# purejade/pinot

Measured on AMD Instinct MI355X. Metric: rows/sec for filter+group-by SUM at 1/2/4/8 GPUs; % of HBM roofline, higher is better.
Workload: dtype int64; 1 GPU; c5: BASELINE configs[4]: 4096 x 2M rows sharded over the GPUs, (f1 IN 32 ids OR f2=7) AND f3<>3, group by gk (card 1000), sum(m); segments=4096, rows_total=8192000000, parallelism=dp1 (segment sharding)

## Files before the change

### pinot_amd/csrc/pgx_roaring.hip

```cpp
#include <hip/hip_runtime.h>
#include <stdint.h>

#include <algorithm>

#include "pgx_device.h"
#include "pgx_internal.h"
#include "pgx_roaring_device.h"

namespace pgx {

__device__ __forceinline__ const PGX_G JRDesc* gdescs(const RDesc* descs) { return (const PGX_G JRDesc*)descs; }

__device__ __forceinline__ PgxRLeavesReg<1> one_leaf(const RDesc* descs, int a) {
  PgxRLeavesReg<1> L;
  L.desc[0] = a;
  L.b0[0] = 0;
  L.total = a >= 0 ? descs[a].nb : 0;
  return L;
}

__global__ void __launch_bounds__(256) pgx_roaring_expand(const RDesc* __restrict__ descs, int npairs, int maxchunks) {
  const int pair = static_cast<int>(blockIdx.x / maxchunks);
  const int chunk = static_cast<int>(blockIdx.x - static_cast<unsigned>(pair) * maxchunks);
  if (pair >= npairs) return;
  const RDesc& D = descs[pair];
  if (chunk >= D.nchunks) return;
  __shared__ uint32_t m[2048];
  __shared__ PgxRScratch S;
  const int tid = threadIdx.x;
  pgx_rexpand<256>(one_leaf(descs, pair), gdescs(descs), chunk, m, S);
  uint32_t* out = D.mask + static_cast<size_t>(chunk) * 2048;
  for (int i = tid; i < 2048; i += 256) out[i] = m[i];
}

constexpr int kRProgStack = 4;
__global__ void __launch_bounds__(256) pgx_roaring_program(const RProg* __restrict__ progs, const RDesc* __restrict__ descs,
                                                           int nprogs, int maxchunks) {
  const int pi = static_cast<int>(blockIdx.x / maxchunks);
  const int chunk = static_cast<int>(blockIdx.x - static_cast<unsigned>(pi) * maxchunks);
  if (pi >= nprogs) return;
  const RProg& P = progs[pi];
  if (chunk >= P.nchunks) return;
  __shared__ uint32_t stk[kRProgStack][2048];
  __shared__ PgxRScratch S;
  const int tid = threadIdx.x;
  const int64_t doc0 = static_cast<int64_t>(chunk) << 16;
  int sp = 0;
  for (int i = 0; i < P.nops; ++i) {
    const int op = P.op[i];
    if (op == RP_LEAF) {
      pgx_rexpand<256>(one_leaf(descs, P.arg[i]), gdescs(descs), chunk, stk[sp], S);
      ++sp;
    } else if (op == RP_NOT) {
      uint32_t* m = stk[sp - 1];
      for (int w = tid; w < 2048; w += 256) m[w] = ~m[w] & pgx_rkeep(doc0 + 32 * w, P.num_docs);
    } else {
      uint32_t* a = stk[sp - 2];
      const uint32_t* b = stk[sp - 1];
      for (int w = tid; w < 2048; w += 256) a[w] = op == RP_AND ? (a[w] & b[w]) : (a[w] | b[w]);
      --sp;
    }
    __syncthreads();
  }
  uint32_t* out = P.mask + static_cast<size_t>(chunk) * 2048;
  for (int w = tid; w < 2048; w += 256) out[w] = stk[0][w];
}

constexpr int kRProgMaxLeaves = PGX_J_MAX_RLEAVES;
__device__ __forceinline__ uint32_t rprog_word(const RProg& P, const uint32_t* lm, int chunk, int w) {
  uint32_t st[kRProgMaxLeaves];
  int sp = 0, leaf = 0;
  const uint32_t keep = pgx_rkeep((static_cast<int64_t>(chunk) << 16) + 32 * w, P.num_docs);
  for (int i = 0; i < P.nops; ++i) {
    const int op = P.op[i];
    if (op == RP_LEAF) {
      st[sp++] = lm[leaf * 2048 + w];
      ++leaf;
    } else if (op == RP_NOT) {
      st[sp - 1] = ~st[sp - 1] & keep;
    } else {
      st[sp - 2] = op == RP_AND ? (st[sp - 2] & st[sp - 1]) : (st[sp - 2] | st[sp - 1]);
      --sp;
    }
  }
  return st[0];
}

__global__ void __launch_bounds__(256) pgx_roaring_program_wide(const RProg* __restrict__ progs,
                                                                const RDesc* __restrict__ descs, int nprogs,
                                                                int maxchunks) {
  const int pi = static_cast<int>(blockIdx.x / maxchunks);
  const int chunk = static_cast<int>(blockIdx.x - static_cast<unsigned>(pi) * maxchunks);
  if (pi >= nprogs) return;
  const RProg& P = progs[pi];
  if (chunk >= P.nchunks) return;
  extern __shared__ uint32_t lmask[];
  __shared__ PgxRScratch S;
  __shared__ int leaf_desc[kRProgMaxLeaves], leaf_b0[kRProgMaxLeaves + 1], nleaves;
  const int tid = threadIdx.x;
  if (tid == 0) {
    int nl = 0, tot = 0;
    for (int i = 0; i < P.nops; ++i)
      if (P.op[i] == RP_LEAF) {
        const int a = P.arg[i];
        leaf_desc[nl] = a;
        leaf_b0[nl] = tot;
        tot += a >= 0 ? descs[a].nb : 0;
        ++nl;
      }
    leaf_b0[nl] = tot;
    nleaves = nl;
  }
  __syncthreads();
  const PgxRLeavesLds L{leaf_desc, leaf_b0, nleaves, leaf_b0[nleaves]};
  pgx_rexpand<256>(L, gdescs(descs), chunk, lmask, S);
  __syncthreads();
  uint32_t* out = P.mask + static_cast<size_t>(chunk) * 2048;
  for (int w = tid; w < 2048; w += 256) out[w] = rprog_word(P, lmask, chunk, w);
}

constexpr int kSegRThreads = 512;
constexpr int kSegRBitmaps = 512;
__global__ void __launch_bounds__(kSegRThreads, 8) pgx_roaring_program_seg(const RProg* __restrict__ progs,
                                                                        const RDesc* __restrict__ descs, int nprogs,
                                                                        int parts) {
  const int pi = static_cast<int>(blockIdx.x) / parts;
  if (pi >= nprogs) return;
  const RProg& P = progs[pi];
  const int per = (P.nchunks + parts - 1) / parts;
  const int c0 = (static_cast<int>(blockIdx.x) % parts) * per;
  const int c1 = min(P.nchunks, c0 + per);
  if (c0 >= c1) return;
  extern __shared__ uint32_t lmask[];
  __shared__ const uint8_t* cptr[kSegRBitmaps];
  __shared__ int ccard[kSegRBitmaps], cpre[kSegRBitmaps + 1], cleaf[kSegRBitmaps];
  __shared__ int ncont;
  __shared__ int bidx[kSegRBitmaps], nbm;
  const int tid = threadIdx.x;
  int nl = 0, tot = 0, leaf = 0, my_desc = -1, my_first = 0;
  for (int i = 0; i < P.nops; ++i)
    if (P.op[i] == RP_LEAF && nl < kRProgMaxLeaves) {
      const int a = P.arg[i];
      const int nb = a >= 0 ? descs[a].nb : 0;
      if (tid >= tot && tid < tot + nb) {
        leaf = nl;
        my_desc = a;
        my_first = tot;
      }
      tot += nb;
      ++nl;
    }
  PgxRCursor cu;
  if (my_desc >= 0) cu.seek(pgx_rbitmap(gdescs(descs) + my_desc, tid - my_first), c0);
  constexpr int kPer = 4;
  for (int chunk = c0; chunk < c1; ++chunk) {
    for (int i = tid; i < nl * 2048; i += kSegRThreads) lmask[i] = 0u;
    if (tid == 0) ncont = 0;
    pgx_lds_barrier();
    if (cu.key == chunk) {
      const int slot = atomicAdd(&ncont, 1);
      cptr[slot] = cu.ptr();
      ccard[slot] = cu.card;
      cleaf[slot] = leaf;
      cu.advance();
    }
    pgx_lds_barrier();
    const int nc = ncont;
    if (tid < 64) pgx_rcard_prefix<kSegRBitmaps / 64, true>(tid, nc, ccard, cpre, &cpre[kSegRBitmaps], bidx, &nbm);
    pgx_lds_barrier();
    const int ne = cpre[kSegRBitmaps];
    const int nbc = nbm;
    uint32_t bw[2048 / kSegRThreads];
    if (nbc > 0) pgx_rwords_load<kSegRThreads>(cptr[bidx[0]], tid, bw);
    pgx_rspread<kSegRThreads, kPer>(tid, nc, ne, cptr, cpre, cleaf, lmask);
    for (int i = 0; i < nbc; ++i) {
      const int k = bidx[i];
      if (i > 0) pgx_rwords_load<kSegRThreads>(cptr[k], tid, bw);
      pgx_rwords_or<kSegRThreads>(lmask + cleaf[k] * 2048, tid, bw);
    }
    pgx_lds_barrier();
    uint32_t* out = P.mask + static_cast<size_t>(chunk) * 2048;
    for (int w = tid; w < 2048; w += kSegRThreads) out[w] = rprog_word(P, lmask, chunk, w);
    pgx_lds_barrier();
  }
}

#ifndef PGX_WAVE_ELEMS
#define PGX_WAVE_ELEMS 16
#endif

template <int NS, int WPB, int MINW>
__global__ void __launch_bounds__(64 * WPB, MINW) pgx_roaring_program_wave(const RProg* __restrict__ progs,
                                                                          const RDesc* __restrict__ descs, int nprogs,
                                                                          int parts) {
  extern __shared__ uint32_t wmask[];
  __shared__ int wpre[WPB][65];
  __shared__ const uint8_t* wptr[WPB][64];
  __shared__ int wslot[WPB][64];
  const int lane = static_cast<int>(threadIdx.x) & 63, wv = static_cast<int>(threadIdx.x) >> 6;
  const int gw = static_cast<int>(blockIdx.x) * WPB + wv;
  const int pi = gw / parts;
  if (pi >= nprogs) return;
  const RProg& P = progs[pi];
  const int per = (P.nchunks + parts - 1) / parts;
  const int c0 = (gw % parts) * per;
  const int c1 = min(P.nchunks, c0 + per);
  if (c0 >= c1) return;
  uint32_t* sm = wmask + wv * NS * 2048;
  int* pre = wpre[wv];
  const uint8_t** ptrs = wptr[wv];
  int* slots = wslot[wv];
  int my_desc = -1, my_first = 0, my_slot = 0, my_phase = 0;
  bool any_andnot = false;
  {
    RPlan plan;
    int tot = 0;
    for (int i = 0; i < P.nops;) {
      const bool is_leaf = P.op[i] == RP_LEAF;
      const int a = P.arg[i];
      i += plan.step(P, i);
      if (!is_leaf) continue;
      const int nb = a >= 0 ? descs[a].nb : 0;
      if (lane >= tot && lane < tot + nb) {
        my_desc = a;
        my_first = tot;
        my_slot = plan.slot;
        my_phase = plan.phase;
      }
      tot += nb;
      any_andnot |= plan.phase != 0;
    }
  }
  PgxRCursor cu;
  if (my_desc >= 0) cu.seek(pgx_rbitmap(gdescs(descs) + my_desc, lane - my_first), c0);
#pragma unroll
  for (int s = 0; s < NS; ++s)
    for (int j = 0; j < 32; ++j) sm[s * 2048 + j * 64 + lane] = 0u;
  for (int chunk = c0; chunk < c1; ++chunk) {
    const bool act = cu.key == chunk;
    const uint8_t* cptr = cu.ptr();
    const int ccard = cu.card;
    if (act) cu.advance();
    for (int ph = 0; ph < (any_andnot ? 2 : 1); ++ph) {
      const bool mine = act && my_phase == ph;
      const bool arr = mine && ccard <= 4096;
      const int v = arr ? ccard : 0;
      int incl = v;
#pragma unroll
      for (int d = 1; d < 64; d <<= 1) {
        const int y = __shfl_up(incl, d, 64);
        if (lane >= d) incl += y;
      }
      const int total = __shfl(incl, 63, 64);
      pre[lane] = incl - v;
      if (lane == 63) pre[64] = incl;
      ptrs[lane] = mine ? cptr : nullptr;
      slots[lane] = my_slot;
      uint64_t bm = __ballot(mine && ccard > 4096);
      pgx_wave_lds_sync();
      if (total > 0) {
        int k = 0;
#pragma unroll
        for (int step = 32; step > 0; step >>= 1)
          if (pre[k + step] <= lane) k += step;
        int kend = pre[k + 1], kbeg = pre[k];
        const uint8_t* kp = ptrs[k];
        int ks = slots[k];
        constexpr int B = PGX_WAVE_ELEMS;
        for (int e0 = lane; e0 < total; e0 += 64 * B) {
          uint32_t val[B];
          int dst[B];
#pragma unroll
          for (int q = 0; q < B; ++q) {
            const int e = e0 + 64 * q;
            dst[q] = -1;
            if (e < total) {
              while (kend <= e) {
                ++k;
                kbeg = kend;
                kend = pre[k + 1];
                kp = ptrs[k];
                ks = slots[k];
              }
              val[q] = pgx_rd16(kp + 2 * (e - kbeg));
              dst[q] = ks * 2048;
            }
          }
#pragma unroll
          for (int q = 0; q < B; ++q)
            if (dst[q] >= 0) {
              if (ph == 0) atomicOr(&sm[dst[q] + (val[q] >> 5)], 1u << (val[q] & 31u));
              else atomicAnd(&sm[dst[q] + (val[q] >> 5)], ~(1u << (val[q] & 31u)));
            }
        }
      }
      while (bm) {
        const int src = __builtin_ctzll(bm);
        bm &= bm - 1;
        const uint8_t* c = ptrs[src];
        uint32_t* m = sm + slots[src] * 2048;
        const bool al = (reinterpret_cast<uintptr_t>(c) & 3u) == 0;
#pragma unroll 1
        for (int h = 0; h < 2; ++h) {
          uint32_t x[16];
          if (al) {
            const PGX_G uint32_t* c32 = (const PGX_G uint32_t*)(c);
#pragma unroll
            for (int j = 0; j < 16; ++j) x[j] = c32[(h * 16 + j) * 64 + lane];
          } else {
#pragma unroll
            for (int j = 0; j < 16; ++j) x[j] = pgx_rd32(c + 4 * ((h * 16 + j) * 64 + lane));
          }
#pragma unroll
          for (int j = 0; j < 16; ++j)
            if (x[j]) {
              if (ph == 0) atomicOr(&m[(h * 16 + j) * 64 + lane], x[j]);
              else atomicAnd(&m[(h * 16 + j) * 64 + lane], ~x[j]);
            }
        }
      }
      pgx_wave_lds_sync();
    }
    const int64_t doc0 = static_cast<int64_t>(chunk) << 16;
    uint32_t* out = P.mask + static_cast<size_t>(chunk) * 2048;
    RPlan plan;
    for (int i = 0; i < P.nops;) {
      const int op = P.op[i];
      i += plan.step(P, i);
      if (op == RP_LEAF) continue;
      uint32_t* a = sm + plan.slot * 2048;
      if (op == RP_NOT) {
#pragma unroll 4
        for (int j = 0; j < 32; ++j) {
          const int w = j * 64 + lane;
          a[w] = ~a[w] & pgx_rkeep(doc0 + 32 * w, P.num_docs);
        }
      } else {
        const uint32_t* b = sm + plan.rhs * 2048;
        if (op == RP_AND) {
#pragma unroll 8
          for (int j = 0; j < 32; ++j) a[j * 64 + lane] &= b[j * 64 + lane];
        } else {
#pragma unroll 8
          for (int j = 0; j < 32; ++j) a[j * 64 + lane] |= b[j * 64 + lane];
        }
      }
    }
    const uint32_t* r = sm + plan.top() * 2048;
#pragma unroll 8
    for (int j = 0; j < 32; ++j) out[j * 64 + lane] = r[j * 64 + lane];
    for (int s = 0; s < NS; ++s)
#pragma unroll 8
      for (int j = 0; j < 32; ++j) sm[s * 2048 + j * 64 + lane] = 0u;
    pgx_wave_lds_sync();
  }
}

}

extern "C" hipError_t pgx_launch_roaring(const pgx::RDesc* descs, int npairs, int maxchunks, hipStream_t stream) {
  if (npairs <= 0 || maxchunks <= 0) return hipSuccess;
  const long long blocks = static_cast<long long>(npairs) * maxchunks;
  if (blocks > 0x7FFFFFFFll) return hipErrorInvalidValue;
  hipLaunchKernelGGL(pgx::pgx_roaring_expand, dim3(static_cast<unsigned>(blocks)), dim3(256), 0, stream, descs, npairs,
                     maxchunks);
  return hipGetLastError();
}

extern "C" hipError_t pgx_launch_roaring_program_wave(const pgx::RProg* progs, const pgx::RDesc* descs, int nprogs,
                                                      int maxchunks, int nslots, hipStream_t stream) {
  if (nprogs <= 0 || maxchunks <= 0) return hipSuccess;
  int parts = std::max(1, std::min(maxchunks, (8192 + nprogs - 1) / nprogs));
  const long long waves = static_cast<long long>(nprogs) * parts;
#define PGX_WAVE_LAUNCH(NS, WPB, MINW)                                                                             \
  hipLaunchKernelGGL((pgx::pgx_roaring_program_wave<NS, WPB, MINW>),                                              \
                     dim3(static_cast<unsigned>((waves + WPB - 1) / WPB)), dim3(64 * WPB),                        \
                     static_cast<size_t>(NS) * WPB * 2048 * 4, stream, progs, descs, nprogs, parts)
  if (nslots <= 1) PGX_WAVE_LAUNCH(1, 4, 4);
  else if (nslots == 2) PGX_WAVE_LAUNCH(2, 2, 2);
  else PGX_WAVE_LAUNCH(3, 2, 1);
#undef PGX_WAVE_LAUNCH
  return hipGetLastError();
}

extern "C" hipError_t pgx_launch_roaring_program(const pgx::RProg* progs, const pgx::RDesc* descs, int nprogs,
                                                 int maxchunks, int maxleaves, hipStream_t stream) {
  if (nprogs <= 0 || maxchunks <= 0) return hipSuccess;
  const long long blocks = static_cast<long long>(nprogs) * maxchunks;
  if (maxleaves < 0 && -maxleaves <= pgx::kRProgMaxLeaves) {
    int parts = std::max(1, std::min(std::min(maxchunks, 8), (2048 + nprogs - 1) / nprogs));
      hipLaunchKernelGGL(pgx::pgx_roaring_program_seg, dim3(static_cast<unsigned>(nprogs * parts)),
                       dim3(pgx::kSegRThreads), static_cast<size_t>(-maxleaves) * 2048 * 4, stream, progs, descs,
                       nprogs, parts);
    return hipGetLastError();
  }
  if (maxleaves >= 1 && maxleaves <= pgx::kRProgMaxLeaves) {
    hipLaunchKernelGGL(pgx::pgx_roaring_program_wide, dim3(static_cast<unsigned>(blocks)), dim3(256),
                       static_cast<size_t>(maxleaves) * 2048 * 4, stream, progs, descs, nprogs, maxchunks);
    return hipGetLastError();
  }
  hipLaunchKernelGGL(pgx::pgx_roaring_program, dim3(static_cast<unsigned>(blocks)), dim3(256), 0, stream, progs, descs,
                     nprogs, maxchunks);
  return hipGetLastError();
}
```

### pinot_amd/csrc/pgx_roaring_device.h

```cpp
#ifndef PGX_ROARING_DEVICE_H_
#define PGX_ROARING_DEVICE_H_

__device__ __forceinline__ u32 pgx_rd16(const unsigned char* p) { return *(const PGX_G unsigned short*)p; }
__device__ __forceinline__ u32 pgx_rd32(const unsigned char* p) { return pgx_rd16(p) | (pgx_rd16(p + 2) << 16); }
__device__ __forceinline__ const unsigned char* pgx_rbitmap(const PGX_G JRDesc* d, int k) {
  const u32 id = ((const PGX_G u32*)d->ids)[k];
  return d->inv + __builtin_bswap32(((const PGX_G u32*)d->inv)[id]);
}

__device__ __forceinline__ int pgx_rcontainer(const unsigned char* base, int chunk, const unsigned char*& ptr) {
  const int n = (int)pgx_rd32(base + 4);
  int lo = 0, hi = n - 1, found = -1;
  const int g = min(chunk, n - 1);
  if (g >= 0) {
    const int k = (int)pgx_rd16(base + 8 + 4 * g);
    if (k == chunk) found = g;
    else if (k < chunk) lo = g + 1;
    else hi = g - 1;
  }
  while (found < 0 && lo <= hi) {
    const int mid = (lo + hi) >> 1;
    const int k = (int)pgx_rd16(base + 8 + 4 * mid);
    if (k == chunk) { found = mid; break; }
    if (k < chunk) lo = mid + 1; else hi = mid - 1;
  }
  if (found < 0) return 0;
  ptr = base + pgx_rd32(base + 8 + 4 * n + 4 * found);
  return (int)pgx_rd16(base + 8 + 4 * found + 2) + 1;
}

struct PgxRCursor {
  const unsigned char* base = nullptr;
  int n = 0, cur = 0, key = 1 << 30, card = 0;
  u32 off = 0;
  __device__ __forceinline__ void load() {
    int k = 1 << 30, c = card;
    u32 o = off;
    if (cur < n) {
      k = (int)pgx_rd16(base + 8 + 4 * cur);
      c = (int)pgx_rd16(base + 8 + 4 * cur + 2) + 1;
      o = pgx_rd32(base + 8 + 4 * n + 4 * cur);
    }
    key = k, card = c, off = o;
  }
  __device__ __forceinline__ void seek(const unsigned char* bitmap, int c0) {
    base = bitmap;
    n = (int)pgx_rd32(base + 4);
    if (c0 > 0 && n > 0) {
      if (n > c0 && (int)pgx_rd16(base + 8 + 4 * c0) == c0) {
        cur = c0;
      } else {
        int lo = 0, hi = n;
        while (lo < hi) {
          const int mid = (lo + hi) >> 1;
          if ((int)pgx_rd16(base + 8 + 4 * mid) < c0) lo = mid + 1; else hi = mid;
        }
        cur = lo;
      }
    }
    load();
  }
  __device__ __forceinline__ void advance() {
    ++cur;
    load();
  }
  __device__ __forceinline__ const unsigned char* ptr() const { return base + off; }
};

template <int PER, bool LIST>
__device__ __forceinline__ void pgx_rcard_prefix(int lane, int nc, const int* ccard, int* cpre, int* total, int* bidx,
                                                 int* nbm) {
  int v[PER], x = 0, nb = 0;
#pragma unroll
  for (int q = 0; q < PER; ++q) {
    const int k = lane * PER + q;
    const bool in = k < nc;
    v[q] = (in && ccard[k] <= 4096) ? ccard[k] : 0;
    if (LIST) nb += (in && ccard[k] > 4096) ? 1 : 0;
    x += v[q];
  }
  int incl = x, binc = nb;
#pragma unroll
  for (int d = 1; d < 64; d <<= 1) {
    const int y = __shfl_up(incl, d, 64);
    const int z = LIST ? __shfl_up(binc, d, 64) : 0;
    if (lane >= d) {
      incl += y;
      binc += z;
    }
  }
  int e = incl - x, b = binc - nb;
#pragma unroll
  for (int q = 0; q < PER; ++q) {
    const int k = lane * PER + q;
    cpre[k] = e;
    e += v[q];
    if (LIST && k < nc && ccard[k] > 4096) bidx[b++] = k;
  }
  if (lane == 63) {
    *total = incl;
    if (LIST) *nbm = binc;
  }
}

template <int NT, int PER>
__device__ __forceinline__ void pgx_rspread(int tid, int nc, int ne, const unsigned char* const* cptr, const int* cpre,
                                            const int* cleaf, u32* lm) {
  for (int e0 = 0; e0 < ne; e0 += PER * NT) {
    u32 val[PER];
    int dst[PER];
#pragma unroll
    for (int q = 0; q < PER; ++q) {
      const int i = e0 + q * NT + tid, e = min(i, ne - 1);
      int lo = 0, hi = nc - 1;
      while (lo < hi) {
        const int mid = (lo + hi + 1) >> 1;
        if (cpre[mid] <= e) lo = mid; else hi = mid - 1;
      }
      val[q] = pgx_rd16(cptr[lo] + 2 * (e - cpre[lo]));
      dst[q] = i < ne ? cleaf[lo] * 2048 : -1;
    }
#pragma unroll
    for (int q = 0; q < PER; ++q) {
      const bool in = dst[q] >= 0;
      atomicOr(&lm[in ? dst[q] + (val[q] >> 5) : tid], in ? 1u << (val[q] & 31u) : 0u);
    }
  }
}

template <int NT>
__device__ __forceinline__ void pgx_rwords_load(const unsigned char* c, int tid, u32* x) {
#pragma unroll
  for (int q = 0; q < 2048 / NT; ++q) x[q] = pgx_rd32(c + 4 * (q * NT + tid));
}
template <int NT>
__device__ __forceinline__ void pgx_rwords_or(u32* m, int tid, const u32* x) {
#pragma unroll
  for (int q = 0; q < 2048 / NT; ++q)
    if (x[q]) atomicOr(&m[q * NT + tid], x[q]);
}

__device__ __forceinline__ u32 pgx_rkeep(long long d, int num_docs) {
  return d >= num_docs ? 0u : (d + 32 > num_docs ? (1u << (num_docs - d)) - 1u : 0xFFFFFFFFu);
}

#define PGX_RB 256
struct PgxRScratch {
  const unsigned char* cptr[PGX_RB];
  int ccard[PGX_RB], cpre[PGX_RB], cleaf[PGX_RB];
  int ncont, celems;
};

template <int NL>
struct PgxRLeavesReg {
  int desc[NL], b0[NL], total;
  __device__ __forceinline__ int leaves() const { return NL; }
  __device__ __forceinline__ void locate(int b, int& leaf, int& d, int& first) const {
    leaf = 0, d = desc[0], first = 0;
#pragma unroll
    for (int q = 1; q < NL; ++q)
      if (b >= b0[q]) { leaf = q; d = desc[q]; first = b0[q]; }
  }
};
struct PgxRLeavesLds {
  const int* desc;
  const int* b0;
  int nl, total;
  __device__ __forceinline__ int leaves() const { return nl; }
  __device__ __forceinline__ void locate(int b, int& leaf, int& d, int& first) const {
    leaf = 0;
    while (b0[leaf + 1] <= b) ++leaf;
    d = desc[leaf], first = b0[leaf];
  }
};

template <int NT, class LT>
__device__ void pgx_rexpand(const LT& L, const PGX_G JRDesc* D, int chunk, u32* lm, PgxRScratch& S) {
  const int tid = threadIdx.x;
  for (int i = tid; i < L.leaves() * 2048; i += NT) lm[i] = 0u;
  for (int b0 = 0; b0 < L.total; b0 += PGX_RB) {
    if (tid == 0) S.ncont = 0;
    pgx_lds_barrier();
    const int b = b0 + tid;
    if (tid < PGX_RB && b < L.total) {
      int leaf, d, first;
      L.locate(b, leaf, d, first);
      const unsigned char* ptr;
      const int card = pgx_rcontainer(pgx_rbitmap(D + d, b - first), chunk, ptr);
      if (card) {
        const int slot = atomicAdd(&S.ncont, 1);
        S.cptr[slot] = ptr;
        S.ccard[slot] = card;
        S.cleaf[slot] = leaf;
      }
    }
    pgx_lds_barrier();
    const int nc = S.ncont;
    if (tid < 64) pgx_rcard_prefix<PGX_RB / 64, false>(tid, nc, S.ccard, S.cpre, &S.celems, nullptr, nullptr);
    pgx_lds_barrier();
    pgx_rspread<NT, 4>(tid, nc, S.celems, S.cptr, S.cpre, S.cleaf, lm);
    for (int k = 0; k < nc; ++k) {
      if (S.ccard[k] <= 4096) continue;
      u32 x[2048 / NT];
      pgx_rwords_load<NT>(S.cptr[k], tid, x);
      pgx_rwords_or<NT>(lm + S.cleaf[k] * 2048, tid, x);
    }
    pgx_lds_barrier();
  }
}

template <int NT, int NL>
__device__ void pgx_rchunk_leaves(const PGX_G JRProg* P, const PGX_G JRDesc* D, int chunk, u32* lm, PgxRScratch& S) {
  PgxRLeavesReg<NL> L;
  L.total = 0;
#pragma unroll
  for (int j = 0; j < NL; ++j) {
    L.desc[j] = P->ldesc[j];
    L.b0[j] = L.total;
    L.total += L.desc[j] >= 0 ? D[L.desc[j]].nb : 0;
  }
  pgx_rexpand<NT>(L, D, chunk, lm, S);
}

#endif
```

Baseline: 1493 billion rows/s.

## Add wide vectorized path to roaring program wave kernel

Adds a WIDE variant of the per-wave roaring program kernel and makes it the default. Array containers are now read as 16-byte granules with per-lane valid masks, and bitmap containers are loaded as 128-bit vectors and realigned with alignbit and shuffles. The prefix sum uses DPP, and the boolean program is evaluated with vector LDS ops. The cursor packs key and card into a single 32-bit load, and parts is now sized from the device CU count. These changes aim to cut scalar 16-bit loads and per-element overhead in mask construction, at the cost of more complexity and register pressure, plus possible alignment edge cases.

```diff
diff --git a/pinot_amd/csrc/pgx_roaring.hip b/pinot_amd/csrc/pgx_roaring.hip
--- a/pinot_amd/csrc/pgx_roaring.hip
+++ b/pinot_amd/csrc/pgx_roaring.hip
@@ -2,6 +2,8 @@
 #include <stdint.h>
 
 #include <algorithm>
+#include <cstdlib>
+#include <cstring>
 
 #include "pgx_device.h"
 #include "pgx_internal.h"
@@ -157,10 +159,10 @@
     for (int i = tid; i < nl * 2048; i += kSegRThreads) lmask[i] = 0u;
     if (tid == 0) ncont = 0;
     pgx_lds_barrier();
-    if (cu.key == chunk) {
+    if (cu.key() == chunk) {
       const int slot = atomicAdd(&ncont, 1);
       cptr[slot] = cu.ptr();
-      ccard[slot] = cu.card;
+      ccard[slot] = cu.card();
       cleaf[slot] = leaf;
       cu.advance();
     }
@@ -185,20 +187,101 @@
   }
 }
 
-#ifndef PGX_WAVE_ELEMS
-#define PGX_WAVE_ELEMS 16
-#endif
-
-template <int NS, int WPB, int MINW>
+constexpr int kWaveGranules = 7;
+constexpr int kWaveNarrowElems = 16;
+typedef u32 pgx_u32x4_dw __attribute__((ext_vector_type(4), aligned(4)));
+
+template <int B>
+__device__ __forceinline__ void wave_granules_load(int base, int end, int lane, const int* pre,
+                                                   const uint8_t* const* ptrs, const int* meta, pgx_u32x4 (&A)[B],
+                                                   u32 (&am)[B]) {
+#pragma unroll
+  for (int q = 0; q < B; ++q) {
+    const int gi = base + 64 * q + lane, g = min(gi, end - 1);
+    int k = 0;
+#pragma unroll
+    for (int step = 32; step > 0; step >>= 1)
+      if (pre[k + step] <= g) k += step;
+    const uintptr_t s = reinterpret_cast<uintptr_t>(ptrs[k]);
+    const int m = meta[k];
+    const uintptr_t ga = (s & ~static_cast<uintptr_t>(15)) + 16 * static_cast<uintptr_t>(g - pre[k]);
+    A[q] = *(const PGX_G pgx_u32x4*)ga;
+    const int first = max(static_cast<int>(s - ga), 0) >> 1;
+    const int last = min(static_cast<int>(s + 2 * (m & 0xFFFF) - ga), 16) >> 1;
+    const u32 vm = gi < end ? (0xFFu >> (8 - last)) & (0xFFu << first) & 0xFFu : 0u;
+    am[q] = vm | static_cast<u32>(m >> 16) << 8;
+  }
+}
+template <int PH, int B>
+__device__ __forceinline__ void wave_granules_apply(u32* sm, const pgx_u32x4 (&A)[B], const u32 (&am)[B]) {
+#pragma unroll
+  for (int q = 0; q < B; ++q) {
+    u32* d = sm + (am[q] >> 8);
+#pragma unroll
+    for (int i = 0; i < 8; ++i) {
+      const u32 w = A[q][i >> 1];
+      const u32 v = (i & 1) ? w >> 16 : w & 0xFFFFu;
+      if ((am[q] >> i) & 1u) {
+        if (PH == 0) atomicOr(&d[v >> 5], 1u << (v & 31u));
+        else atomicAnd(&d[v >> 5], ~(1u << (v & 31u)));
+      }
+    }
+  }
+}
+template <int J0, int H>
+__device__ __forceinline__ void wave_words_load(uintptr_t c, int lane, pgx_u32x4 (&W)[H], u32& tail) {
+  const PGX_G unsigned char* cb = (const PGX_G unsigned char*)(c & ~static_cast<uintptr_t>(3));
+#pragma unroll
+  for (int j = 0; j < H; ++j) W[j] = *(const PGX_G pgx_u32x4_dw*)(cb + static_cast<u32>(16 * (64 * (J0 + j) + lane)));
+  tail = 0u;
+  if ((c & 2) && lane == 0) tail = *(const PGX_G u32*)(cb + 1024u * (J0 + H));
+}
+template <int PH, int J0, int H>
+__device__ __forceinline__ void wave_words_apply(u32* m, uintptr_t c, int lane, const pgx_u32x4 (&W)[H], u32 tail) {
+  const u32 sh = (c & 2) ? 16u : 0u;
+  pgx_u32x4* m4 = reinterpret_cast<pgx_u32x4*>(m) + 64 * J0 + lane;
+#pragma unroll
+  for (int j = 0; j < H; ++j) {
+    const u32 wrap = __builtin_amdgcn_readfirstlane(j < H - 1 ? W[(j + 1) % H].x : tail);
+    const u32 up = __shfl(W[j].x, (lane + 1) & 63, 64);
+    const u32 next = lane == 63 ? wrap : up;
+    pgx_u32x4 o;
+    o.x = __builtin_amdgcn_alignbit(W[j].y, W[j].x, sh);
+    o.y = __builtin_amdgcn_alignbit(W[j].z, W[j].y, sh);
+    o.z = __builtin_amdgcn_alignbit(W[j].w, W[j].z, sh);
+    o.w = __builtin_amdgcn_alignbit(next, W[j].w, sh);
+    const pgx_u32x4 cur = m4[64 * j];
+    m4[64 * j] = PH == 0 ? (cur | o) : (cur & ~o);
+  }
+}
+__device__ __forceinline__ int wave_prefix_sum(int v) {
+  v += __builtin_amdgcn_update_dpp(0, v, 0x111, 0xF, 0xF, false);
+  v += __builtin_amdgcn_update_dpp(0, v, 0x112, 0xF, 0xF, false);
+  v += __builtin_amdgcn_update_dpp(0, v, 0x114, 0xF, 0xF, false);
+  v += __builtin_amdgcn_update_dpp(0, v, 0x118, 0xF, 0xF, false);
+  v += __builtin_amdgcn_update_dpp(0, v, 0x142, 0xA, 0xF, false);
+  v += __builtin_amdgcn_update_dpp(0, v, 0x143, 0xC, 0xF, false);
+  return v;
+}
+__device__ __forceinline__ int wave_bits_below(uint64_t m) {
+  return static_cast<int>(__builtin_amdgcn_mbcnt_hi(static_cast<u32>(m >> 32), __builtin_amdgcn_mbcnt_lo(static_cast<u32>(m), 0u)));
+}
+__device__ __forceinline__ uintptr_t wave_lane_ptr(uintptr_t v, int src) {
+  const u32 lo = __builtin_amdgcn_readlane(static_cast<u32>(v), src);
+  const u32 hi = __builtin_amdgcn_readlane(static_cast<u32>(v >> 32), src);
+  return (static_cast<uintptr_t>(hi) << 32) | lo;
+}
+
+template <int NS, int WPB, int MINW, bool WIDE>
 __global__ void __launch_bounds__(64 * WPB, MINW) pgx_roaring_program_wave(const RProg* __restrict__ progs,
                                                                           const RDesc* __restrict__ descs, int nprogs,
                                                                           int parts) {
-  extern __shared__ uint32_t wmask[];
+  extern __shared__ __attribute__((aligned(16))) uint32_t wmask[];
   __shared__ int wpre[WPB][65];
   __shared__ const uint8_t* wptr[WPB][64];
   __shared__ int wslot[WPB][64];
   const int lane = static_cast<int>(threadIdx.x) & 63, wv = static_cast<int>(threadIdx.x) >> 6;
-  const int gw = static_cast<int>(blockIdx.x) * WPB + wv;
+  const int gw = __builtin_amdgcn_readfirstlane(static_cast<int>(blockIdx.x) * WPB + wv);
   const int pi = gw / parts;
   if (pi >= nprogs) return;
   const RProg& P = progs[pi];
@@ -207,11 +290,13 @@
   const int c1 = min(P.nchunks, c0 + per);
   if (c0 >= c1) return;
   uint32_t* sm = wmask + wv * NS * 2048;
+  pgx_u32x4* sm4 = reinterpret_cast<pgx_u32x4*>(sm);
   int* pre = wpre[wv];
   const uint8_t** ptrs = wptr[wv];
   int* slots = wslot[wv];
   int my_desc = -1, my_first = 0, my_slot = 0, my_phase = 0;
-  bool any_andnot = false;
+  bool any_andnot = false, rest = false;
+  int top_slot = 0;
   {
     RPlan plan;
     int tot = 0;
@@ -219,6 +304,8 @@
       const bool is_leaf = P.op[i] == RP_LEAF;
       const int a = P.arg[i];
       i += plan.step(P, i);
+      top_slot = plan.top();
+      rest |= !is_leaf;
       if (!is_leaf) continue;
       const int nb = a >= 0 ? descs[a].nb : 0;
       if (lane >= tot && lane < tot + nb) {
@@ -236,11 +323,126 @@
 #pragma unroll
   for (int s = 0; s < NS; ++s)
     for (int j = 0; j < 32; ++j) sm[s * 2048 + j * 64 + lane] = 0u;
+  const bool out16 = (reinterpret_cast<uintptr_t>(P.mask) & 15u) == 0;
   for (int chunk = c0; chunk < c1; ++chunk) {
-    const bool act = cu.key == chunk;
+    const bool act = cu.key() == chunk;
     const uint8_t* cptr = cu.ptr();
-    const int ccard = cu.card;
+    const int ccard = cu.card();
     if (act) cu.advance();
+    if constexpr (WIDE) {
+      constexpr int B = kWaveGranules;
+      const uintptr_t cs = reinterpret_cast<uintptr_t>(cptr);
+      const bool arr = act && ccard <= 4096, p1 = my_phase != 0;
+      const int ng = arr ? static_cast<int>(((cs + 2 * ccard - 1) >> 4) - (cs >> 4)) + 1 : 0;
+      const u32 v = p1 ? static_cast<u32>(ng) << 16 : static_cast<u32>(ng);
+      const u32 incl = static_cast<u32>(wave_prefix_sum(static_cast<int>(v)));
+      const u32 tot = __builtin_amdgcn_readlane(incl, 63);
+      const int t0 = static_cast<int>(tot & 0xFFFFu), t = t0 + static_cast<int>(tot >> 16);
+      const uint64_t a0 = __ballot(arr && !p1), a1 = __ballot(arr && p1);
+      const int n0 = __popcll(a0), na = n0 + __popcll(a1);
+      if (arr) {
+        const int rank = p1 ? n0 + wave_bits_below(a1) : wave_bits_below(a0);
+        pre[rank] = p1 ? t0 + static_cast<int>((incl - v) >> 16) : static_cast<int>((incl - v) & 0xFFFFu);
+        ptrs[rank] = cptr;
+        slots[rank] = ccard | (my_slot * 2048) << 16;
+      }
+      if (lane >= na) pre[lane] = t;
+      if (lane == 63) pre[64] = t;
+      uint64_t b0 = __ballot(act && !arr && !p1), b1 = __ballot(act && !arr && p1);
+      pgx_wave_lds_sync();
+      pgx_u32x4 A[B], W0[4];
+      u32 am[B], tail0 = 0u;
+#pragma unroll
+      for (int j = 0; j < 4; ++j) W0[j] = pgx_u32x4{0u, 0u, 0u, 0u};
+      const int held = b0 ? __builtin_ctzll(b0) : (b1 ? __builtin_ctzll(b1) : -1);
+      if (t0 > 0) {
+        wave_granules_load<B>(0, t0, lane, pre, ptrs, slots, A, am);
+        if (held >= 0) wave_words_load<0, 4>(wave_lane_ptr(cs, held), lane, W0, tail0);
+        for (int base = 0;;) {
+          wave_granules_apply<0, B>(sm, A, am);
+          base += 64 * B;
+          if (base >= t0) break;
+          wave_granules_load<B>(base, t0, lane, pre, ptrs, slots, A, am);
+        }
+      } else if (held >= 0) {
+        wave_words_load<0, 4>(wave_lane_ptr(cs, held), lane, W0, tail0);
+      }
+      while (b0) {
+        const int src = __builtin_ctzll(b0);
+        b0 &= b0 - 1;
+        const uintptr_t c = wave_lane_ptr(cs, src);
+        u32* m = sm + __builtin_amdgcn_readlane(my_slot, src) * 2048;
+        pgx_u32x4 W1[4];
+        u32 tail1;
+        if (src != held) wave_words_load<0, 4>(c, lane, W0, tail0);
+        wave_words_load<4, 4>(c, lane, W1, tail1);
+        wave_words_apply<0, 0, 4>(m, c, lane, W0, tail0);
+        wave_words_apply<0, 4, 4>(m, c, lane, W1, tail1);
+      }
+      if (t > t0 || b1) {
+        pgx_wave_lds_sync();
+        while (b1) {
+          const int src = __builtin_ctzll(b1);
+          b1 &= b1 - 1;
+          const uintptr_t c = wave_lane_ptr(cs, src);
+          u32* m = sm + __builtin_amdgcn_readlane(my_slot, src) * 2048;
+          pgx_u32x4 W1[4];
+          u32 tail1;
+          if (src != held) wave_words_load<0, 4>(c, lane, W0, tail0);
+          wave_words_load<4, 4>(c, lane, W1, tail1);
+          wave_words_apply<1, 0, 4>(m, c, lane, W0, tail0);
+          wave_words_apply<1, 4, 4>(m, c, lane, W1, tail1);
+        }
+        for (int base = t0; base < t; base += 64 * B) {
+          wave_granules_load<B>(base, t, lane, pre, ptrs, slots, A, am);
+          wave_granules_apply<1, B>(sm, A, am);
+        }
+      }
+      pgx_wave_lds_sync();
+      const int64_t doc0 = static_cast<int64_t>(chunk) << 16;
+      RPlan plan;
+      for (int i = 0; rest && i < P.nops;) {
+        const int op = P.op[i];
+        i += plan.step(P, i);
+        if (op == RP_LEAF) continue;
+        pgx_u32x4* a = sm4 + plan.slot * 512;
+        if (op == RP_NOT) {
+#pragma unroll 2
+          for (int j = 0; j < 8; ++j) {
+            const int w = 4 * (64 * j + lane);
+            pgx_u32x4 x = a[64 * j + lane];
+            x.x = ~x.x & pgx_rkeep(doc0 + 32 * w, P.num_docs);
+            x.y = ~x.y & pgx_rkeep(doc0 + 32 * (w + 1), P.num_docs);
+            x.z = ~x.z & pgx_rkeep(doc0 + 32 * (w + 2), P.num_docs);
+            x.w = ~x.w & pgx_rkeep(doc0 + 32 * (w + 3), P.num_docs);
+            a[64 * j + lane] = x;
+          }
+        } else {
+          const pgx_u32x4* b = sm4 + plan.rhs * 512;
+          if (op == RP_AND) {
+#pragma unroll
+            for (int j = 0; j < 8; ++j) a[64 * j + lane] &= b[64 * j + lane];
+          } else {
+#pragma unroll
+            for (int j = 0; j < 8; ++j) a[64 * j + lane] |= b[64 * j + lane];
+          }
+        }
+      }
+      const pgx_u32x4* r = sm4 + top_slot * 512;
+      PGX_G uint32_t* out = (PGX_G uint32_t*)P.mask + static_cast<size_t>(chunk) * 2048;
+      if (out16) {
+#pragma unroll
+        for (int j = 0; j < 8; ++j) ((PGX_G pgx_u32x4*)out)[64 * j + lane] = r[64 * j + lane];
+      } else {
+#pragma unroll
+        for (int j = 0; j < 8; ++j) ((PGX_G pgx_u32x4_dw*)out)[64 * j + lane] = r[64 * j + lane];
+      }
+      for (int s = 0; s < NS; ++s)
+#pragma unroll
+        for (int j = 0; j < 8; ++j) sm4[s * 512 + 64 * j + lane] = pgx_u32x4{0u, 0u, 0u, 0u};
+      pgx_wave_lds_sync();
+      continue;
+    }
     for (int ph = 0; ph < (any_andnot ? 2 : 1); ++ph) {
       const bool mine = act && my_phase == ph;
       const bool arr = mine && ccard <= 4096;
@@ -266,7 +468,7 @@
         int kend = pre[k + 1], kbeg = pre[k];
         const uint8_t* kp = ptrs[k];
         int ks = slots[k];
-        constexpr int B = PGX_WAVE_ELEMS;
+        constexpr int B = kWaveNarrowElems;
         for (int e0 = lane; e0 < total; e0 += 64 * B) {
           uint32_t val[B];
           int dst[B];
@@ -367,18 +569,55 @@
   return hipGetLastError();
 }
 
+namespace {
+struct WaveKnobs {
+  bool narrow = false;
+  int parts = 0;
+};
+WaveKnobs wave_knobs() {
+  WaveKnobs k;
+  const char* e = std::getenv("PGX_DEBUG");
+  while (e && *e) {
+    const char* end = std::strchr(e, ',');
+    const size_t n = end ? static_cast<size_t>(end - e) : std::strlen(e);
+    if (n == 7 && std::strncmp(e, "rnarrow", 7) == 0) k.narrow = true;
+    else if (n > 7 && std::strncmp(e, "rparts=", 7) == 0) k.parts = std::atoi(e + 7);
+    e = end ? end + 1 : nullptr;
+  }
+  return k;
+}
+int device_cus() {
+  static const int cus = [] {
+    int dev = 0, n = 0;
+    if (hipGetDevice(&dev) != hipSuccess ||
+        hipDeviceGetAttribute(&n, hipDeviceAttributeMultiprocessorCount, dev) != hipSuccess || n <= 0)
+      n = 256;
+    return n;
+  }();
+  return cus;
+}
+}
+
 extern "C" hipError_t pgx_launch_roaring_program_wave(const pgx::RProg* progs, const pgx::RDesc* descs, int nprogs,
                                                       int maxchunks, int nslots, hipStream_t stream) {
   if (nprogs <= 0 || maxchunks <= 0) return hipSuccess;
-  int parts = std::max(1, std::min(maxchunks, (8192 + nprogs - 1) / nprogs));
+  const WaveKnobs kn = wave_knobs();
+  const int target = 2 * 16 * device_cus();
+  int parts = std::max(1, std::min(maxchunks, kn.parts > 0 ? kn.parts : (target + nprogs - 1) / nprogs));
   const long long waves = static_cast<long long>(nprogs) * parts;
-#define PGX_WAVE_LAUNCH(NS, WPB, MINW)                                                                             \
-  hipLaunchKernelGGL((pgx::pgx_roaring_program_wave<NS, WPB, MINW>),                                              \
+#define PGX_WAVE_LAUNCH(NS, WPB, MINW, WIDE)                                                                       \
+  hipLaunchKernelGGL((pgx::pgx_roaring_program_wave<NS, WPB, MINW, WIDE>),                                        \
                      dim3(static_cast<unsigned>((waves + WPB - 1) / WPB)), dim3(64 * WPB),                        \
                      static_cast<size_t>(NS) * WPB * 2048 * 4, stream, progs, descs, nprogs, parts)
-  if (nslots <= 1) PGX_WAVE_LAUNCH(1, 4, 4);
-  else if (nslots == 2) PGX_WAVE_LAUNCH(2, 2, 2);
-  else PGX_WAVE_LAUNCH(3, 2, 1);
+  if (kn.narrow) {
+    if (nslots <= 1) PGX_WAVE_LAUNCH(1, 4, 4, false);
+    else if (nslots == 2) PGX_WAVE_LAUNCH(2, 2, 2, false);
+    else PGX_WAVE_LAUNCH(3, 2, 1, false);
+  } else {
+    if (nslots <= 1) PGX_WAVE_LAUNCH(1, 4, 4, true);
+    else if (nslots == 2) PGX_WAVE_LAUNCH(2, 2, 2, true);
+    else PGX_WAVE_LAUNCH(3, 2, 1, true);
+  }
 #undef PGX_WAVE_LAUNCH
   return hipGetLastError();
 }
diff --git a/pinot_amd/csrc/pgx_roaring_device.h b/pinot_amd/csrc/pgx_roaring_device.h
--- a/pinot_amd/csrc/pgx_roaring_device.h
+++ b/pinot_amd/csrc/pgx_roaring_device.h
@@ -31,18 +31,18 @@
 
 struct PgxRCursor {
   const unsigned char* base = nullptr;
-  int n = 0, cur = 0, key = 1 << 30, card = 0;
-  u32 off = 0;
+  int n = 0, cur = 0;
+  u32 kc = 0, off = 0;
   __device__ __forceinline__ void load() {
-    int k = 1 << 30, c = card;
-    u32 o = off;
+    u32 k = kc, o = off;
     if (cur < n) {
-      k = (int)pgx_rd16(base + 8 + 4 * cur);
-      c = (int)pgx_rd16(base + 8 + 4 * cur + 2) + 1;
+      k = pgx_rd32(base + 8 + 4 * cur);
       o = pgx_rd32(base + 8 + 4 * n + 4 * cur);
     }
-    key = k, card = c, off = o;
-  }
+    kc = k, off = o;
+  }
+  __device__ __forceinline__ int key() const { return cur < n ? (int)(kc & 0xFFFFu) : 1 << 30; }
+  __device__ __forceinline__ int card() const { return (int)(kc >> 16) + 1; }
   __device__ __forceinline__ void seek(const unsigned char* bitmap, int c0) {
     base = bitmap;
     n = (int)pgx_rd32(base + 4);
```

Result: faster. 1525 billion rows/s, median of 6 (+2.2%).
